# soedinglab/hh-suite

Hardware: NVIDIA H100
Metric: Viterbi GCUPS (query_L x sum target_L / s) (higher is better)
Workload: dtype f32

## Files before the change

### hh-suite_b200/csrc/hhg_api.cu

```cuda
#include "../../include/hhg.h"
#include "hhg_kernels.cuh"
#include "hhg_hhm.cuh"
#include "hhg_msa.cuh"
#include "hhg_crf.cuh"
#include "hhg_mac.cuh"
#include "hhg_topk.cuh"
#include "hhg_hitlist.h"

#include <dlfcn.h>
#if defined(__SSE__)
#include <xmmintrin.h>
#endif

#include <algorithm>
#include <chrono>
#include <atomic>
#include <cstdarg>
#include <cstdio>
#include <cstdlib>
#include <cstring>
#include <memory>
#include <cmath>
#include <cfloat>
#include <mutex>
// ... 82 lines not shown
}

}

struct hhg_ctx {
  int device = 0;
  std::shared_ptr<void> msa_cache;
  std::shared_ptr<void> crf_cache;
  std::shared_ptr<void> msa_rcp;
  cudaStream_t stream = nullptr;
  bool own_stream = false;
  int sm_count = 0;
  long long launches = 0;
  int Lq = 0, R = 0;
  int nq = 0;
  std::vector<int> q_L, q_row0;
  std::vector<float> h_q_pav;
  bool has_q_pav = false;
  DevBuf<float> d_q_pav, d_pb;
  std::vector<int> ex;
  int ex_nq = 0, ex_nt = 0;
  DevBuf<int> d_ex;
  unsigned long long query_serial = 0;
  int group_jobs = 16;
  uint32_t epoch = 0;
  uint32_t epoch_window = 1;
  DevBuf<float4> qrec;
  DevBuf<float> S33;
  DevBuf<float> lg2, diff;
  std::vector<float> h_lg2;
  bool has_ss = false, has_S33 = false;
  hhg_params par{1, 0.f, 0.f, -0.03f, 0.11f, 0, 0.1f, 2};
  DevBuf<uint8_t> pf_prof, sw_prof;
  DevBuf<uint8_t> pf_edge[2];
  DevBuf<int> sw_ids, sw_scores;
  DevBuf<unsigned> pf_counter, pf_hist;
  DevBuf<int> pf_corr, pf_ids_a, pf_score_a, pf_ids_b;
  int mac_Lq = 0;
  DevBuf<float> mac_qp, mac_qtr, mac_ttr, mac_post, mac_out_post;
  DevBuf<uint8_t> mac_off, mac_bt, mac_out_states;
  DevBuf<double> mac_rows, mac_scale;
  DevBuf<long long> mac_i64, mac_dbg;
  DevBuf<int> mac_i32, mac_out_i, mac_out_j, mac_map;
  cudaStream_t aux_stream = nullptr;
  cudaEvent_t aux_ev[2] = {nullptr, nullptr};
  DevBuf<MacHitOut> mac_out;
  std::vector<long long> mac_cell_off;
// ... 113 lines not shown
  c->device = device;
  c->sm_count = prop.multiProcessorCount;
  if (stream) {
    c->stream = (cudaStream_t)stream;
  } else {
    CK(cudaStreamCreateWithFlags(&c->stream, cudaStreamNonBlocking));
    c->own_stream = true;
  }
  c->R = strip_rows();
  {
    std::vector<float> lg2(1025, 0.f), diff(1025, 0.f);
    float prev = 0.0f;
    for (int i = 1; i <= 1024; ++i) {
      lg2[i] = (float)(::log((double)(1024 + i)) * 1.442695041 - 10.0);
      diff[i - 1] = (float)((double)(lg2[i] - prev) * 1.2352E-4);
      prev = lg2[i];
    }
    c->h_lg2 = lg2;
    cudaError_t e1 = c->lg2.alloc(1025), e2 = c->diff.alloc(1025);
    if (e1 != cudaSuccess || e2 != cudaSuccess) return fail(HHG_ENOMEM, "fast_log2 tables");
    CK(cudaMemcpy(c->lg2.p, lg2.data(), 1025 * 4, cudaMemcpyHostToDevice));
    CK(cudaMemcpy(c->diff.p, diff.data(), 1025 * 4, cudaMemcpyHostToDevice));
  }
  { const char* ge = getenv("HHG_GROUP_JOBS"); c->group_jobs = ge ? std::max(1, atoi(ge)) : 16; }
  size_t free_b = 0, total_b = 0;
  CK(cudaMemGetInfo(&free_b, &total_b));
  const char* env = getenv("HHG_MAX_BT_GB");
  double cap = env ? atof(env) * 1e9 : 48e9;
  c->max_bt_bytes = (size_t)std::min(cap, 0.45 * (double)free_b);
  *out = holder.release();
  return HHG_OK;
}

int hhg_ctx_destroy(hhg_ctx* ctx) {
  if (!ctx) return HHG_OK;
  cudaSetDevice(ctx->device);
  if (ctx->scratch_plan) hhg_plan_destroy(ctx->scratch_plan);
  for (auto& e : ctx->ev) if (e) cudaEventDestroy(e);
  for (auto& e : ctx->aux_ev) if (e) cudaEventDestroy(e);
  if (ctx->aux_stream) cudaStreamDestroy(ctx->aux_stream);
  if (ctx->own_stream && ctx->stream) cudaStreamDestroy(ctx->stream);
  delete ctx;
  return HHG_OK;
}

int hhg_ctx_sync(hhg_ctx* ctx) {
  if (!ctx) return fail(HHG_EINVAL, "ctx is NULL");
// ... 1149 lines not shown
      max_wave_words = std::max(max_wave_words, wave_bt);
      w.job_begin = jb;
      wave_bt = 0;
    }
    JobDesc d{};
    d.ss_off = ss; d.bt_off = (long long)wave_bt; d.bnd_off = bnd; d.co_off = co; d.jc_off = jc;
    d.Lmax = Lmax; d.query = q; d.nstrips = ns; d.Lq = ctx->q_L[q]; d.qrow0 = ctx->q_row0[q];
    pl->jobs.push_back(d);
    wave_bt += words;
    bnd += (long long)(Lmax + 1) * 32;
    jc += (long long)Lmax * 224;
    co += (long long)ns * (Lmax + 1) * 32;
    ss += ns;
    pl->padded_cells += (double)ns * R * (double)Lmax * 32.0;
    first += cnt;
  }
  pl->njobs = (int)pl->jobs.size();
  w.job_end = pl->njobs;
  pl->waves.push_back(w);
  max_wave_words = std::max(max_wave_words, wave_bt);
  pl->ss_total = ss;
  pl->co_total = co;
  pl->items.clear();
  for (Wave& wv : pl->waves) {
    wv.item_begin = (long long)pl->items.size();
    for (int g0 = wv.job_begin; g0 < wv.job_end; g0 += ctx->group_jobs) {
      const int g1 = std::min(g0 + ctx->group_jobs, wv.job_end);
      int maxns = 0;
      for (int jb = g0; jb < g1; ++jb) maxns = std::max(maxns, pl->jobs[jb].nstrips);
      for (int sidx = 0; sidx < maxns; ++sidx)
        for (int jb = g0; jb < g1; ++jb)
          if (sidx < pl->jobs[jb].nstrips) pl->items.push_back(make_int2(jb - wv.job_begin, sidx));
    }
    wv.item_end = (long long)pl->items.size();
  }
  long long po = 0;
  double cols_sum = 0;
  for (int k = 0; k < n; ++k) {
    ReqDesc& r = pl->reqs[k];
    r.target = pl->ids[k];
    r.Lt = db->L[r.target];
    r.Lq = ctx->q_L[pl->req_query[k]];
    r.path_off = po;
    po += r.Lq + r.Lt + 2;
    pl->cells += (double)r.Lq * r.Lt;
    cols_sum += r.Lt;
  }
  if (po > 0x7fffffffLL) return fail(HHG_EINVAL, "plan too large: %lld path bytes (> 2^31-1); split the request", po);
  pl->path_total = po;
  pl->jc_total = jc;
  pl->alg_bytes = cols_sum * 112.0 + pl->cells * 1.0 + (double)sizeof(HitRec) * n;

  cudaError_t e = cudaSuccess;
  auto A = [&](cudaError_t r) { if (e == cudaSuccess) e = r; };
  A(pl->d_jobs.ensure(pl->njobs)); A(pl->d_reqs.ensure(n));
  A(pl->d_job_target.ensure(job_target.size())); A(pl->d_items.ensure(pl->items.size()));
  A(pl->d_jcols.ensure((size_t)jc + 224));
// ... 86 lines not shown
    ctx->launches++;
    CK(cudaGetLastError());
    CK(cudaStreamSynchronize(ctx->stream));
  }
  pl->celloff = true;
  pl->n_excl_steps = (int)total;
  return HHG_OK;
}

int hhg_set_excluded_regions(hhg_ctx* ctx, int nq, const int32_t* q_lo, const int32_t* q_hi, int nt, const int32_t* t_lo,
                             const int32_t* t_hi) {
  if (!ctx || nq < 0 || nt < 0 || (nq && (!q_lo || !q_hi)) || (nt && (!t_lo || !t_hi)))
    return fail(HHG_EINVAL, "hhg_set_excluded_regions: bad argument");
  ctx->ex.assign(q_lo, q_lo + nq);
  ctx->ex.insert(ctx->ex.end(), q_hi, q_hi + nq);
  ctx->ex.insert(ctx->ex.end(), t_lo, t_lo + nt);
  ctx->ex.insert(ctx->ex.end(), t_hi, t_hi + nt);
  ctx->ex_nq = nq;
  ctx->ex_nt = nt;
  return HHG_OK;
}

template <int R>
static int launch_viterbi(hhg_ctx* ctx, const VitParams& P, bool local, bool ss, bool co, int items) {
  const size_t smem = (size_t)kWarpsPerCta * (R * 112 + kRingBytes) + 64 + (ss ? 44 * 44 * 4 : 0);
  void (*kern)(const VitParams) = nullptr;
#define PICK(L_, S_, C_) kern = k_viterbi<R, L_, S_, C_>
  if (local) { if (ss) { if (co) PICK(true, true, true); else PICK(true, true, false); }
               else    { if (co) PICK(true, false, true); else PICK(true, false, false); } }
  else       { if (ss) { if (co) PICK(false, true, true); else PICK(false, true, false); }
               else    { if (co) PICK(false, false, true); else PICK(false, false, false); } }
#undef PICK
  CK(cudaFuncSetAttribute(kern, cudaFuncAttributeMaxDynamicSharedMemorySize, (int)smem));
  int per_sm = 0;
  CK(cudaOccupancyMaxActiveBlocksPerMultiprocessor(&per_sm, kern, kWarpsPerCta * 32, smem));
  if (per_sm < 1) return fail(HHG_ECUDA, "viterbi kernel does not fit on an SM");
  int grid = ctx->sm_count * per_sm;
  const int need = (items + kWarpsPerCta - 1) / kWarpsPerCta;
  if (grid > need) grid = need;
  kern<<<grid, kWarpsPerCta * 32, smem, ctx->stream>>>(P);
  ctx->launches++;
  CK(cudaGetLastError());
  return HHG_OK;
}

static int plan_run_impl(hhg_ctx* ctx, hhg_plan* pl, bool timed) {
  if (!ctx || !pl) return fail(HHG_EINVAL, "hhg_plan_run: bad argument");
  if (pl->q_L != ctx->q_L || pl->q_row0 != ctx->q_row0) return fail(HHG_EINVAL, "plan was made for another query (batch) geometry");
  const hhg_db* db = pl->db;
  const bool fused = pl->nm_mode >= 0;
  if (fused && (!db->raw || !ctx->has_q_pav)) return fail(HHG_EINVAL, "fused null model needs a raw shard and query pav");
  if (!fused && !db->prepared) return fail(HHG_EINVAL, "raw db: call hhg_db_apply_null_model for the current query first");
  if (ctx->par.use_ss && (!db->has_ss || !ctx->has_ss || !ctx->has_S33))
    return fail(HHG_EINVAL, "use_ss requested but query/db/S33 carry no ss information");
  CK(cudaSetDevice(ctx->device));
  cudaStream_t st = ctx->stream;
  ctx->epoch = (ctx->epoch + 1) & 0xFFFFFu;
  if (ctx->epoch == 0) { ctx->epoch = 1; ctx->epoch_window++; }
  if (pl->bnd_epoch_window != ctx->epoch_window) {
    if (pl->d_bnd.p) CK(cudaMemsetAsync(pl->d_bnd.p, 0, pl->d_bnd.n * sizeof(BndSlot), st));
    pl->bnd_epoch_window = ctx->epoch_window;
  }
  CK(cudaMemsetAsync(pl->d_counter.p, 0, pl->waves.size() * 4, st));
  if (pl->jc_version != db->cols_version || pl->jc_nm_mode != pl->nm_mode ||
      (fused && pl->jc_query_serial != ctx->query_serial)) {
    int maxL = 0;
    for (const JobDesc& jd : pl->jobs) maxL = std::max(maxL, jd.Lmax);
    dim3 grid((unsigned)pl->njobs, (unsigned)std::min(64, (maxL + 7) / 8), 1);
    k_interleave_cols<<<grid, 256, 0, st>>>(pl->d_jobs.p, pl->d_job_target.p, fused ? db->cols_raw.p : db->cols.p,
                                            db->dcol_off.p, db->dL.p, pl->d_jcols.p, pl->nm_mode, ctx->d_q_pav.p,
                                            db->pav.p, ctx->d_pb.p);
    ctx->launches++;
    CK(cudaGetLastError());
    pl->jc_version = db->cols_version;
    pl->jc_nm_mode = pl->nm_mode;
    pl->jc_query_serial = ctx->query_serial;
  }
  for (size_t wi = 0; wi < pl->waves.size(); ++wi) {
    const Wave& w = pl->waves[wi];
    const int nj = w.job_end - w.job_begin;
    VitParams P{};
    P.qrec = ctx->qrec.p;
    P.jobs = pl->d_jobs.p + w.job_begin;
    P.items = pl->d_items.p + w.item_begin; P.n_items = (int)(w.item_end - w.item_begin);
    P.Lt = db->dL.p;
    P.jcols = pl->d_jcols.p;
    P.njobs = nj;
    P.job_target = pl->d_job_target.p + (size_t)w.job_begin * 32;
    P.bt = pl->d_bt.p; P.bnd = pl->d_bnd.p;
    P.tag_base = ctx->epoch << 12;
    P.counter = pl->d_counter.p + wi;
    P.strip_score = pl->d_strip_score.p;
    P.strip_ij = pl->d_strip_ij.p;
    P.celloff = pl->celloff ? pl->d_co.p : nullptr;
    P.S33 = ctx->has_S33 ? ctx->S33.p : nullptr;
    P.egq = ctx->par.egq; P.egt = ctx->par.egt; P.shift = ctx->par.shift; P.ssw = ctx->par.ssw;
    P.zero = 0u;

    const int items = P.n_items;
    int rc;
    if (timed) CK(cudaEventRecord(ctx->ev[0], st));
    if (pl->R == 8) rc = launch_viterbi<8>(ctx, P, ctx->par.local != 0, ctx->par.use_ss != 0, pl->celloff, items);
    else if (pl->R == 12) rc = launch_viterbi<12>(ctx, P, ctx->par.local != 0, ctx->par.use_ss != 0, pl->celloff, items);
    else rc = launch_viterbi<16>(ctx, P, ctx->par.local != 0, ctx->par.use_ss != 0, pl->celloff, items);
    if (rc != HHG_OK) return rc;
    if (timed) CK(cudaEventRecord(ctx->ev[1], st));
    BtParams B{};
    B.n_req = pl->n;
    B.jobs = pl->d_jobs.p; B.reqs = pl->d_reqs.p;
    B.nm_mode = pl->nm_mode; B.q_pav = ctx->d_q_pav.p; B.t_pav = db->pav.p; B.pb = ctx->d_pb.p;
    B.bt = pl->d_bt.p; B.strip_score = pl->d_strip_score.p; B.strip_ij = pl->d_strip_ij.p;
    B.hits = pl->d_hits.p; B.paths = pl->d_paths.p;
    B.job_begin = w.job_begin; B.job_end = w.job_end;
    B.qrec = ctx->qrec.p; B.cols = fused ? db->cols_raw.p : db->cols.p; B.col_off = db->dcol_off.p;
    B.lg2 = ctx->lg2.p; B.diff = ctx->diff.p; B.S33 = ctx->has_S33 ? ctx->S33.p : nullptr; B.S = pl->d_S.p;
    B.corr = ctx->par.corr; B.ssw = ctx->par.ssw; B.use_ss = ctx->par.use_ss; B.ss_score_mode = (ctx->par.ssm == 2);
    const int threads = 128;
    k_backtrace<<<(pl->n + threads - 1) / threads, threads, 0, st>>>(B);
    ctx->launches++;
    CK(cudaGetLastError());
    if (timed) {
      CK(cudaEventRecord(ctx->ev[2], st));
      CK(cudaEventSynchronize(ctx->ev[2]));
      float a = 0, b = 0;
      CK(cudaEventElapsedTime(&a, ctx->ev[0], ctx->ev[1]));
      CK(cudaEventElapsedTime(&b, ctx->ev[1], ctx->ev[2]));
      pl->ms_viterbi += a;
// ... 851 lines not shown
```

### hh-suite_b200/csrc/hhg_kernels.cuh

```cuda
#pragma once
#include <cuda_runtime.h>
#include <float.h>
#include <stdint.h>

#ifndef HHG_MAX3
#define HHG_MAX3 1
#endif

#include "hhg_math.cuh"

namespace hhg {

constexpr int kWarpsPerCta = 4;

struct __align__(16) ColRec {
  float p[20];
  float m2m, m2d, d2m, d2d, i2m;
  float i2i, m2i;
  uint32_t ss;
};
static_assert(sizeof(ColRec) == 112, "ColRec must be 7 x 16 bytes");

struct __align__(8) BndSlot {
  unsigned long long w[5];
// ... 9 lines not shown
  asm volatile("st.relaxed.gpu.global.v2.b64 [%0], {%1,%2};" ::"l"(p + 2 * lane), "l"(tagged(mm, tag)),
               "l"(tagged(dg, tag)) : "memory");
  asm volatile("st.relaxed.gpu.global.v2.b64 [%0], {%1,%2};" ::"l"(p + 64 + 2 * lane), "l"(tagged(mi, tag)),
               "l"(tagged(gd, tag)) : "memory");
  asm volatile("st.relaxed.gpu.global.b64 [%0], %1;" ::"l"(p + 128 + lane), "l"(tagged(im, tag)) : "memory");
}
__device__ __forceinline__ void ld_slot(const BndSlot* col, int lane, float& mm, float& dg, float& mi, float& gd,
                                        float& im, uint32_t (&tag)[5]) {
  const unsigned long long* p = reinterpret_cast<const unsigned long long*>(col);
  unsigned long long w0, w1, w2, w3, w4;
  asm volatile("ld.relaxed.gpu.global.v2.b64 {%0,%1}, [%2];" : "=l"(w0), "=l"(w1) : "l"(p + 2 * lane) : "memory");
  asm volatile("ld.relaxed.gpu.global.v2.b64 {%0,%1}, [%2];" : "=l"(w2), "=l"(w3) : "l"(p + 64 + 2 * lane) : "memory");
  asm volatile("ld.relaxed.gpu.global.b64 %0, [%1];" : "=l"(w4) : "l"(p + 128 + lane) : "memory");
  mm = __uint_as_float((uint32_t)w0); tag[0] = (uint32_t)(w0 >> 32);
  dg = __uint_as_float((uint32_t)w1); tag[1] = (uint32_t)(w1 >> 32);
  mi = __uint_as_float((uint32_t)w2); tag[2] = (uint32_t)(w2 >> 32);
  gd = __uint_as_float((uint32_t)w3); tag[3] = (uint32_t)(w3 >> 32);
  im = __uint_as_float((uint32_t)w4); tag[4] = (uint32_t)(w4 >> 32);
}
__device__ __forceinline__ bool slot_ok(const uint32_t (&tag)[5], uint32_t want) {
  return ((tag[0] ^ want) | (tag[1] ^ want) | (tag[2] ^ want) | (tag[3] ^ want) | (tag[4] ^ want)) == 0u;
}

struct JobDesc {
  long long ss_off;
  long long bt_off;
  long long bnd_off;
  long long co_off;
  long long jc_off;
  int Lmax;
  int query;
  int nstrips;
  int Lq;
  int qrow0;
};
static_assert(sizeof(JobDesc) == 64, "JobDesc: 5 x int64 + 5 x int32, tail padding only");

struct ReqDesc {
  long long path_off;
  int job;
  int lane;
  int target;
  int Lt;
  int Lq;
};
static_assert(sizeof(ReqDesc) == 32, "ReqDesc: 1 x int64 + 5 x int32, tail padding only");

struct VitParams {
  const float4* qrec;
  const JobDesc* jobs;
  const int2* items;
  int n_items;
  const int* Lt;
  const float4* jcols;
  int njobs;
  const int* job_target;
  uint32_t* bt;
  struct BndSlot* bnd;
  uint32_t tag_base;
  unsigned int* counter;
  float* strip_score;
  int* strip_ij;
  const uint32_t* celloff;
  const float* S33;
  float egq, egt, shift, ssw;
  uint32_t zero;
};

__device__ __forceinline__ uint32_t smem_u32(const void* p) {
// ... 31 lines not shown
  const float e = __fadd_rn(__uint_as_float((u >> 23) | 0x4B000000u), -8388735.0f);
  const float m = __uint_as_float((u & 0x007FFFFFu) | 0x3F800000u);
  float p = -0.107254423828329604454f;
  p = __fadd_rn(__fmul_rn(p, m), 0.688243882994381274313f);
  p = __fadd_rn(__fmul_rn(p, m), -1.75647175389045657003f);
  p = __fadd_rn(__fmul_rn(p, m), 2.61761038894603480148f);
  p = __fmul_rn(p, __fadd_rn(m, -1.0f));
  return __fadd_rn(p, e);
}

__device__ __forceinline__ float dot20_dev(const float4 (&t)[5], const float4 (&q)[5]) {
  float r0 = __fmul_rn(t[0].x, q[0].x), r1 = __fmul_rn(t[0].y, q[0].y);
  float r2 = __fmul_rn(t[0].z, q[0].z), r3 = __fmul_rn(t[0].w, q[0].w);
#pragma unroll
  for (int m = 1; m < 5; ++m) {
    r0 = __fadd_rn(__fmul_rn(t[m].x, q[m].x), r0);
    r1 = __fadd_rn(__fmul_rn(t[m].y, q[m].y), r1);
    r2 = __fadd_rn(__fmul_rn(t[m].z, q[m].z), r2);
    r3 = __fadd_rn(__fmul_rn(t[m].w, q[m].w), r3);
  }
  return __fadd_rn(__fadd_rn(r0, r1), __fadd_rn(r2, r3));
}

__device__ __forceinline__ void cp_async_jc(float4* dst, const float4* src) {
  asm volatile("cp.async.cg.shared.global [%0], [%1], 16;" ::"r"(smem_u32(dst)), "l"(src) : "memory");
}
__device__ __forceinline__ void cp_async_commit() { asm volatile("cp.async.commit_group;" ::: "memory"); }
__device__ __forceinline__ void cp_async_wait_all() { asm volatile("cp.async.wait_all;" ::: "memory"); }

constexpr int kJcSlot = 7 * 32;
constexpr size_t kRingBytes = 2 * kJcSlot * 16;

#define HHG_NEG (-FLT_MAX)

template <int R, bool LOCAL, bool SS, bool CELLOFF>
__global__ void __launch_bounds__(kWarpsPerCta * 32, (R <= 12) ? 3 : 2)
    k_viterbi(const VitParams P) {
  static_assert(R % 4 == 0, "R must be a multiple of 4");
  extern __shared__ __align__(128) unsigned char smem_raw[];
  const int warp = threadIdx.x >> 5;
  const int lane = threadIdx.x & 31;
  float4* qs = reinterpret_cast<float4*>(smem_raw) + (size_t)warp * R * 7;
  constexpr size_t kRingOff = (size_t)kWarpsPerCta * R * 112;
  float4* ring = reinterpret_cast<float4*>(smem_raw + kRingOff + (size_t)warp * kRingBytes) + lane;
  constexpr size_t kBarOff = kRingOff + kWarpsPerCta * kRingBytes;
  uint64_t* bars = reinterpret_cast<uint64_t*>(smem_raw + kBarOff);
  float* s33 = reinterpret_cast<float*>(smem_raw + kBarOff + 64);
  uint64_t* bar = bars + warp;

  if (lane == 0) mbar_init(bar, 1);
  if (SS) {
    for (int k = threadIdx.x; k < 44 * 44; k += blockDim.x) s33[k] = P.S33[k];
  }
  asm volatile("fence.mbarrier_init.release.cluster;" ::: "memory");
  __syncthreads();

  const float smin = LOCAL ? 0.0f : HHG_NEG;
  const int total_items = P.n_items;
  uint32_t parity = 0;

  for (;;) {
    int item = 0;
    if (lane == 0) item = (int)atomicAdd(P.counter, 1u);
    item = __shfl_sync(0xffffffffu, item, 0);
    if (item >= total_items) break;
    const int2 it = __ldg(P.items + item);
    const int job = it.x, s = it.y;
    const JobDesc* jd = P.jobs + job;
    const int Lq = jd->Lq;
    const int nstrips = jd->nstrips;
    const int i0 = s * R;

    if (lane == 0) {
      mbar_expect_tx(bar, R * 112);
      tma_bulk_g2s(qs, P.qrec + (size_t)(jd->qrow0 + i0) * 7, R * 112, bar);
    }

    const int t = P.job_target[job * 32 + lane];
    const int Lt = P.Lt[t];
    const int Lmax = jd->Lmax;
    const float4* jc = P.jcols + jd->jc_off + lane;
    const size_t bt_row_stride = (size_t)(Lmax + 1) * 32;
    uint32_t* btc = P.bt + jd->bt_off + lane + (size_t)(i0 >> 2) * bt_row_stride + 32;
    BndSlot* bndc = P.bnd + jd->bnd_off + 32;
    const uint32_t tag_in = P.tag_base + (uint32_t)s;
    const uint32_t tag_out = P.tag_base + (uint32_t)s + 1u;
    const bool last_strip = (s == nstrips - 1);
    const uint32_t* co = nullptr;
    if (CELLOFF) co = P.celloff + jd->co_off + (size_t)s * (Lmax + 1) * 32 + lane + 32;

    float MM[R], GD[R], IM[R], DG[R], Y[R];
#pragma unroll
    for (int r = 0; r < R; ++r) {
      MM[r] = __fmul_rn((float)(-(i0 + 1 + r)), P.egq);
      GD[r] = IM[r] = DG[r] = HHG_NEG;
    }
    float dtMM = __fmul_rn((float)(-i0), P.egq), dtDG = HHG_NEG, dtGD = HHG_NEG, dtIM = HHG_NEG;

    float best = HHG_NEG;
    int bi = 0, bj = 0;

#pragma unroll
    for (int k = 0; k < 7; ++k) cp_async_jc(ring + k * 32, jc + k * 32);
    cp_async_commit();
    int rd = 0;

    float nMM = 0.f, nDG = 0.f, nMI = 0.f, nGD = 0.f, nIM = 0.f;
    uint32_t ntag[5] = {0u, 0u, 0u, 0u, 0u};
    if (s > 0) ld_slot(bndc, lane, nMM, nDG, nMI, nGD, nIM, ntag);

    mbar_wait(bar, parity);
    parity ^= 1u;
#pragma unroll
    for (int r = 0; r < R; ++r) Y[r] = __fadd_rn(HHG_NEG, qs[r * 7 + 5].x);

    for (int j = 1; j <= Lmax; ++j) {
      cp_async_wait_all();
      const float4* cur = ring + rd;
      const float4 tp[5] = {cur[0], cur[32], cur[64], cur[96], cur[128]};
      const float4 tt0 = cur[160], tt1 = cur[192];
      const float t_m2m = tt0.x, t_m2d = tt0.y, t_d2m = tt0.z, t_d2d = tt0.w;
      const float t_i2m = tt1.x, t_i2i = tt1.y, t_m2i = tt1.z;
      const uint32_t t_ss = __float_as_uint(tt1.w);
      rd ^= kJcSlot;
      jc += 224;
#pragma unroll
      for (int k = 0; k < 7; ++k) cp_async_jc(ring + rd + k * 32, jc + k * 32);
      cp_async_commit();

      float tMM, tDG, tMI, tGD, tIM;
      if (s == 0) {
        tMM = __fmul_rn((float)(-j), P.egt);
        tDG = tMI = tGD = tIM = HHG_NEG;
      } else {
        if (!__all_sync(0xffffffffu, slot_ok(ntag, tag_in))) {
          while (!slot_ok(ntag, tag_in)) {
            __nanosleep(20);
            ld_slot(bndc, lane, nMM, nDG, nMI, nGD, nIM, ntag);
          }
        }
        tMM = nMM; tDG = nDG; tMI = nMI; tGD = nGD; tIM = nIM;
        ld_slot(bndc + 32, lane, nMM, nDG, nMI, nGD, nIM, ntag);
      }
      uint32_t cow = 0;
      if (CELLOFF) cow = __ldg(co);

      float4 qa = qs[5], qb = qs[6];
      float pMM = __fadd_rn(dtMM, qa.x), pGD = __fadd_rn(dtGD, qa.x), pIM = __fadd_rn(dtIM, qb.x),
            pDG = __fadd_rn(dtDG, qa.z);
      float uMM = tMM, uDG = tDG, uMI = tMI;
      const float bcmp = (j <= Lt) ? best : INFINITY;
      float bc = bcmp;

      uint32_t word = SS ? 0u : (t_ss & P.zero);
#pragma unroll
      for (int r = 0; r < R; ++r) {
        float4 q[5];
#pragma unroll
        for (int k = 0; k < 5; ++k) q[k] = qs[r * 7 + k];
        const float q_m2m = qa.x, q_m2d = qa.y, q_d2m = qa.z, q_d2d = qa.w;
        const float q_i2m = qb.x, q_i2i = qb.y, q_m2i = qb.z;

        uint32_t b;
        float mm;
        const float c1 = __fadd_rn(pMM, t_m2m);
        const float c2 = __fadd_rn(pGD, t_d2m);
        const float c3 = __fadd_rn(pIM, t_m2m);
        const float c4 = __fadd_rn(pDG, t_m2m);
        const float c5 = __fadd_rn(Y[r], t_i2m);
#if HHG_MAX3
        mm = fmaxf(fmaxf(smin, c1), c2);
        mm = fmaxf(fmaxf(mm, c3), c4);
        mm = fmaxf(mm, c5);
        b = 6u;
        b = (c4 == mm) ? 5u : b;
        b = (c3 == mm) ? 4u : b;
        b = (c2 == mm) ? 3u : b;
        b = (c1 == mm) ? 2u : b;
        b = (smin == mm) ? 0u : b;
#else
        b = (c1 > smin) ? 2u : 0u; mm = fmaxf(smin, c1);
        b = (c2 > mm) ? 3u : b;    mm = fmaxf(mm, c2);
        b = (c3 > mm) ? 4u : b;    mm = fmaxf(mm, c3);
        b = (c4 > mm) ? 5u : b;    mm = fmaxf(mm, c4);
        b = (c5 > mm) ? 6u : b;    mm = fmaxf(mm, c5);
#endif

        float Si = log2f4_dev(dot20_dev(tp, q));
        if (SS) {
          const uint32_t q_ss = __float_as_uint(qb.w);
          Si = __fadd_rn(__fmul_rn(P.ssw, s33[q_ss * 44 + t_ss]), Si);
        }
        Si = __fadd_rn(Si, P.shift);
        mm = __fadd_rn(mm, Si);

        const float oMM = MM[r], oGD = GD[r], oIM = IM[r], oDG = DG[r];
        float a1, a2, gd, im, dg, mi;
        a1 = __fadd_rn(oMM, t_m2d); a2 = __fadd_rn(oGD, t_d2d);
        b |= (a1 > a2) ? 8u : 0u;  gd = fmaxf(a1, a2);
        a1 = __fadd_rn(__fadd_rn(oMM, q_m2i), t_m2m); a2 = __fadd_rn(__fadd_rn(oIM, q_i2i), t_m2m);
        b |= (a1 > a2) ? 16u : 0u; im = fmaxf(a1, a2);
        a1 = __fadd_rn(uMM, q_m2d); a2 = __fadd_rn(uDG, q_d2d);
        b |= (a1 > a2) ? 32u : 0u; dg = fmaxf(a1, a2);
        Y[r] = __fadd_rn(uMI, q_m2m);
        a1 = __fadd_rn(__fadd_rn(uMM, q_m2m), t_m2i); a2 = __fadd_rn(Y[r], t_i2i);
        b |= (a1 > a2) ? 64u : 0u; mi = fmaxf(a1, a2);

        if (CELLOFF) {
          const float off = ((cow >> r) & 1u) ? HHG_NEG : 0.0f;
          mm = __fadd_rn(mm, off); gd = __fadd_rn(gd, off); im = __fadd_rn(im, off);
          dg = __fadd_rn(dg, off); mi = __fadd_rn(mi, off);
        }

        word |= b << (8 * (r & 3));
        if ((r & 3) == 3) {
          __stcs(btc + (size_t)(r >> 2) * bt_row_stride, word);
          word = 0;
        }
        if (r + 1 < R) {
          qa = qs[(r + 1) * 7 + 5]; qb = qs[(r + 1) * 7 + 6];
          pMM = __fadd_rn(oMM, qa.x); pGD = __fadd_rn(oGD, qa.x); pIM = __fadd_rn(oIM, qb.x);
          pDG = __fadd_rn(oDG, qa.z);
        }
        uMM = mm; uDG = dg; uMI = mi;
        MM[r] = mm; GD[r] = gd; IM[r] = im; DG[r] = dg;
      }
      dtMM = tMM; dtDG = tDG; dtGD = tGD; dtIM = tIM;

      {
        float c0 = MM[0], c1 = MM[1], c2 = MM[2], c3 = MM[3];
#pragma unroll
        for (int r = 4; r < R; r += 4) {
          c0 = fmaxf(c0, MM[r]); c1 = fmaxf(c1, MM[r + 1]); c2 = fmaxf(c2, MM[r + 2]); c3 = fmaxf(c3, MM[r + 3]);
        }
        if (fmaxf(fmaxf(c0, c1), fmaxf(c2, c3)) >= bc) {
#pragma unroll
          for (int r = 0; r < R; ++r) {
            const float mm = MM[r];
            if (mm >= bc) {
              const int i = i0 + 1 + r;
              const bool cand = (i <= Lq) && (LOCAL || i == Lq || j == Lt);
              if (cand && (mm > best || i < bi)) { best = mm; bi = i; bj = j; bc = mm; }
            }
          }
        }
      }

      if (!last_strip) st_slot(bndc, lane, uMM, uDG, uMI, GD[R - 1], IM[R - 1], tag_out);
      bndc += 32;
      btc += 32;
      if (CELLOFF) co += 32;
    }
    int jb = job;
    asm("" : "+r"(jb));
    const size_t o = ((size_t)P.jobs[jb].ss_off + s) * 32 + lane;
    P.strip_score[o] = best;
    P.strip_ij[o] = (bi << 16) | bj;
    cp_async_wait_all();
    __syncwarp();
  }
}

__device__ __forceinline__ void null_model_vec(int columnscore, const float* __restrict__ q_pav,
                                               const float* __restrict__ t_pav, const float* __restrict__ pb,
                                               float (&pn)[20]) {
#pragma unroll
  for (int a = 0; a < 20; ++a) {
    switch (columnscore) {
      case 0: pn[a] = pb[a]; break;
      case 2: pn[a] = t_pav[a]; break;
      case 3: pn[a] = q_pav[a]; break;
      default: pn[a] = __fmul_rn(0.5f, __fadd_rn(q_pav[a], t_pav[a])); break;
    }
  }
}
__device__ __forceinline__ float4 div4(float4 v, const float* pn) {
  v.x = __fdiv_rn(v.x, pn[0]); v.y = __fdiv_rn(v.y, pn[1]); v.z = __fdiv_rn(v.z, pn[2]); v.w = __fdiv_rn(v.w, pn[3]);
  return v;
}

struct HitRec {
  float score;
// ... 462 lines not shown
```

Measured before the change: 191.6.

## Hand off strip boundaries between warps via shared-memory mbarrier rings

Work is now scheduled per CTA in quads of consecutive strips of the same job. Adjacent warps pass boundary column values through a shared-memory ring guarded by mbarriers, replacing the global-memory tagged boundary slots and polling. The plan builder groups strips into CTA-sized runs with padding, the default group size rises from 16 to 256, and cp.async switches from .cg to .ca. The cost is extra shared memory per CTA, possible idle warps from padding, and a __syncthreads per quad that ties warps together.

```diff
diff --git a/hh-suite_b200/csrc/hhg_api.cu b/hh-suite_b200/csrc/hhg_api.cu
--- a/hh-suite_b200/csrc/hhg_api.cu
+++ b/hh-suite_b200/csrc/hhg_api.cu
@@ -128,7 +128,7 @@
   int ex_nq = 0, ex_nt = 0;
   DevBuf<int> d_ex;
   unsigned long long query_serial = 0;
-  int group_jobs = 16;
+  int group_jobs = 256;
   uint32_t epoch = 0;
   uint32_t epoch_window = 1;
   DevBuf<float4> qrec;
@@ -288,7 +288,7 @@
     CK(cudaMemcpy(c->lg2.p, lg2.data(), 1025 * 4, cudaMemcpyHostToDevice));
     CK(cudaMemcpy(c->diff.p, diff.data(), 1025 * 4, cudaMemcpyHostToDevice));
   }
-  { const char* ge = getenv("HHG_GROUP_JOBS"); c->group_jobs = ge ? std::max(1, atoi(ge)) : 16; }
+  { const char* ge = getenv("HHG_GROUP_JOBS"); c->group_jobs = ge ? std::max(1, atoi(ge)) : 256; }
   size_t free_b = 0, total_b = 0;
   CK(cudaMemGetInfo(&free_b, &total_b));
   const char* env = getenv("HHG_MAX_BT_GB");
@@ -1484,17 +1484,31 @@
   pl->ss_total = ss;
   pl->co_total = co;
   pl->items.clear();
+  auto push_run = [&](int jb, int s0, int cnt) {
+    for (int k = 0; k < cnt; ++k)
+      pl->items.push_back(make_int2(jb, (s0 + k) | (k > 0 ? kFromWarp : 0) | (k + 1 < cnt ? kToWarp : 0)));
+  };
+  auto pad_quad = [&] {
+    while (pl->items.size() % kWarpsPerCta) pl->items.push_back(make_int2(-1, 0));
+  };
   for (Wave& wv : pl->waves) {
-    wv.item_begin = (long long)pl->items.size();
+    wv.item_begin = (long long)pl->items.size() / kWarpsPerCta;
     for (int g0 = wv.job_begin; g0 < wv.job_end; g0 += ctx->group_jobs) {
       const int g1 = std::min(g0 + ctx->group_jobs, wv.job_end);
-      int maxns = 0;
-      for (int jb = g0; jb < g1; ++jb) maxns = std::max(maxns, pl->jobs[jb].nstrips);
-      for (int sidx = 0; sidx < maxns; ++sidx)
+      int maxq = 0;
+      for (int jb = g0; jb < g1; ++jb) maxq = std::max(maxq, pl->jobs[jb].nstrips / kWarpsPerCta);
+      for (int q = 0; q < maxq; ++q)
         for (int jb = g0; jb < g1; ++jb)
-          if (sidx < pl->jobs[jb].nstrips) pl->items.push_back(make_int2(jb - wv.job_begin, sidx));
+          if (q < pl->jobs[jb].nstrips / kWarpsPerCta) push_run(jb - wv.job_begin, q * kWarpsPerCta, kWarpsPerCta);
+      for (int jb = g0; jb < g1; ++jb) {
+        const int ns = pl->jobs[jb].nstrips, rem = ns % kWarpsPerCta;
+        if (rem == 0) continue;
+        if ((int)(pl->items.size() % kWarpsPerCta) + rem > kWarpsPerCta) pad_quad();
+        push_run(jb - wv.job_begin, ns - rem, rem);
+      }
+      pad_quad();
     }
-    wv.item_end = (long long)pl->items.size();
+    wv.item_end = (long long)pl->items.size() / kWarpsPerCta;
   }
   long long po = 0;
   double cols_sum = 0;
@@ -1627,8 +1641,8 @@
 }
 
 template <int R>
-static int launch_viterbi(hhg_ctx* ctx, const VitParams& P, bool local, bool ss, bool co, int items) {
-  const size_t smem = (size_t)kWarpsPerCta * (R * 112 + kRingBytes) + 64 + (ss ? 44 * 44 * 4 : 0);
+static int launch_viterbi(hhg_ctx* ctx, const VitParams& P, bool local, bool ss, bool co, int quads) {
+  const size_t smem = vit_smem_bytes(R, ss);
   void (*kern)(const VitParams) = nullptr;
 #define PICK(L_, S_, C_) kern = k_viterbi<R, L_, S_, C_>
   if (local) { if (ss) { if (co) PICK(true, true, true); else PICK(true, true, false); }
@@ -1641,8 +1655,7 @@
   CK(cudaOccupancyMaxActiveBlocksPerMultiprocessor(&per_sm, kern, kWarpsPerCta * 32, smem));
   if (per_sm < 1) return fail(HHG_ECUDA, "viterbi kernel does not fit on an SM");
   int grid = ctx->sm_count * per_sm;
-  const int need = (items + kWarpsPerCta - 1) / kWarpsPerCta;
-  if (grid > need) grid = need;
+  if (grid > quads) grid = quads;
   kern<<<grid, kWarpsPerCta * 32, smem, ctx->stream>>>(P);
   ctx->launches++;
   CK(cudaGetLastError());
@@ -1687,7 +1700,7 @@
     VitParams P{};
     P.qrec = ctx->qrec.p;
     P.jobs = pl->d_jobs.p + w.job_begin;
-    P.items = pl->d_items.p + w.item_begin; P.n_items = (int)(w.item_end - w.item_begin);
+    P.items = pl->d_items.p + w.item_begin * kWarpsPerCta; P.n_items = (int)(w.item_end - w.item_begin);
     P.Lt = db->dL.p;
     P.jcols = pl->d_jcols.p;
     P.njobs = nj;
@@ -1702,12 +1715,12 @@
     P.egq = ctx->par.egq; P.egt = ctx->par.egt; P.shift = ctx->par.shift; P.ssw = ctx->par.ssw;
     P.zero = 0u;
 
-    const int items = P.n_items;
+    const int quads = P.n_items;
     int rc;
     if (timed) CK(cudaEventRecord(ctx->ev[0], st));
-    if (pl->R == 8) rc = launch_viterbi<8>(ctx, P, ctx->par.local != 0, ctx->par.use_ss != 0, pl->celloff, items);
-    else if (pl->R == 12) rc = launch_viterbi<12>(ctx, P, ctx->par.local != 0, ctx->par.use_ss != 0, pl->celloff, items);
-    else rc = launch_viterbi<16>(ctx, P, ctx->par.local != 0, ctx->par.use_ss != 0, pl->celloff, items);
+    if (pl->R == 8) rc = launch_viterbi<8>(ctx, P, ctx->par.local != 0, ctx->par.use_ss != 0, pl->celloff, quads);
+    else if (pl->R == 12) rc = launch_viterbi<12>(ctx, P, ctx->par.local != 0, ctx->par.use_ss != 0, pl->celloff, quads);
+    else rc = launch_viterbi<16>(ctx, P, ctx->par.local != 0, ctx->par.use_ss != 0, pl->celloff, quads);
     if (rc != HHG_OK) return rc;
     if (timed) CK(cudaEventRecord(ctx->ev[1], st));
     BtParams B{};
diff --git a/hh-suite_b200/csrc/hhg_kernels.cuh b/hh-suite_b200/csrc/hhg_kernels.cuh
--- a/hh-suite_b200/csrc/hhg_kernels.cuh
+++ b/hh-suite_b200/csrc/hhg_kernels.cuh
@@ -55,6 +55,19 @@
   return ((tag[0] ^ want) | (tag[1] ^ want) | (tag[2] ^ want) | (tag[3] ^ want) | (tag[4] ^ want)) == 0u;
 }
 
+constexpr int kHandCols = 8;
+struct HandCol {
+  float4 a[32];
+  float b[32];
+};
+struct HandRing {
+  HandCol col[kHandCols];
+  uint64_t full[kHandCols], empty[kHandCols];
+};
+static_assert(sizeof(HandRing) == 5248, "HandRing: 8 x 640 B columns + 16 mbarriers");
+__host__ __device__ constexpr uint32_t hand_full(uint32_t c) { return kHandCols * sizeof(HandCol) + 8 * c; }
+__host__ __device__ constexpr uint32_t hand_empty(uint32_t c) { return (kHandCols * sizeof(HandCol)) + 8 * (kHandCols + c); }
+
 struct JobDesc {
   long long ss_off;
   long long bt_off;
@@ -78,6 +91,10 @@
   int Lq;
 };
 static_assert(sizeof(ReqDesc) == 32, "ReqDesc: 1 x int64 + 5 x int32, tail padding only");
+
+constexpr int kFromWarp = 1 << 30;
+constexpr int kToWarp = 1 << 29;
+constexpr int kStripMask = kToWarp - 1;
 
 struct VitParams {
   const float4* qrec;
@@ -155,14 +172,42 @@
   return __fadd_rn(__fadd_rn(r0, r1), __fadd_rn(r2, r3));
 }
 
+__device__ __forceinline__ bool mbar_test_a(uint32_t bar, uint32_t parity) {
+  uint32_t ok;
+  asm volatile("{ .reg .pred p; mbarrier.test_wait.parity.shared::cta.b64 p, [%1], %2; selp.u32 %0, 1, 0, p; }"
+               : "=r"(ok) : "r"(bar), "r"(parity) : "memory");
+  return ok != 0;
+}
+__device__ __forceinline__ void mbar_wait_a(uint32_t bar, uint32_t parity) {
+  while (!mbar_test_a(bar, parity)) __nanosleep(20);
+}
+__device__ __forceinline__ void mbar_arrive_a(uint32_t bar) {
+  asm volatile("mbarrier.arrive.shared::cta.b64 _, [%0];" ::"r"(bar) : "memory");
+}
+__device__ __forceinline__ void hand_put(uint32_t col, int lane, float mm, float dg, float mi, float gd, float im) {
+  asm volatile("st.shared.v4.f32 [%0], {%1,%2,%3,%4};" ::"r"(col + 16 * lane), "f"(mm), "f"(dg), "f"(mi), "f"(gd)
+               : "memory");
+  asm volatile("st.shared.f32 [%0], %1;" ::"r"(col + 512 + 4 * lane), "f"(im) : "memory");
+}
+__device__ __forceinline__ void hand_get(uint32_t col, int lane, float& mm, float& dg, float& mi, float& gd, float& im) {
+  asm volatile("ld.shared.v4.f32 {%0,%1,%2,%3}, [%4];" : "=f"(mm), "=f"(dg), "=f"(mi), "=f"(gd) : "r"(col + 16 * lane)
+               : "memory");
+  asm volatile("ld.shared.f32 %0, [%1];" : "=f"(im) : "r"(col + 512 + 4 * lane) : "memory");
+}
+
 __device__ __forceinline__ void cp_async_jc(float4* dst, const float4* src) {
-  asm volatile("cp.async.cg.shared.global [%0], [%1], 16;" ::"r"(smem_u32(dst)), "l"(src) : "memory");
+  asm volatile("cp.async.ca.shared.global [%0], [%1], 16;" ::"r"(smem_u32(dst)), "l"(src) : "memory");
 }
 __device__ __forceinline__ void cp_async_commit() { asm volatile("cp.async.commit_group;" ::: "memory"); }
 __device__ __forceinline__ void cp_async_wait_all() { asm volatile("cp.async.wait_all;" ::: "memory"); }
 
 constexpr int kJcSlot = 7 * 32;
 constexpr size_t kRingBytes = 2 * kJcSlot * 16;
+
+__host__ __device__ constexpr size_t vit_smem_bytes(int R, bool ss) {
+  return (size_t)kWarpsPerCta * (R * 112 + kRingBytes) + 64 + (kWarpsPerCta - 1) * sizeof(HandRing) +
+         (ss ? 44 * 44 * 4 : 0);
+}
 
 #define HHG_NEG (-FLT_MAX)
 
@@ -178,10 +223,21 @@
   float4* ring = reinterpret_cast<float4*>(smem_raw + kRingOff + (size_t)warp * kRingBytes) + lane;
   constexpr size_t kBarOff = kRingOff + kWarpsPerCta * kRingBytes;
   uint64_t* bars = reinterpret_cast<uint64_t*>(smem_raw + kBarOff);
-  float* s33 = reinterpret_cast<float*>(smem_raw + kBarOff + 64);
+  volatile int* quad_idx = reinterpret_cast<volatile int*>(smem_raw + kBarOff + 32);
+  HandRing* hands = reinterpret_cast<HandRing*>(smem_raw + kBarOff + 64);
+  float* s33 = reinterpret_cast<float*>(hands + (kWarpsPerCta - 1));
   uint64_t* bar = bars + warp;
+  HandRing* hin = reinterpret_cast<HandRing*>(smem_raw + kBarOff + 64 - sizeof(HandRing)) + warp;
+  const uint32_t hin_a = smem_u32(hin);
+  uint32_t hin_n = 0, hout_n = 0;
 
   if (lane == 0) mbar_init(bar, 1);
+  if (threadIdx.x < (kWarpsPerCta - 1) * kHandCols) {
+    HandRing& h = hands[threadIdx.x / kHandCols];
+    mbar_init(&h.full[threadIdx.x % kHandCols], 32);
+    mbar_init(&h.empty[threadIdx.x % kHandCols], 32);
+  }
+  if (threadIdx.x == 0) quad_idx[0] = (int)atomicAdd(P.counter, 1u);
   if (SS) {
     for (int k = threadIdx.x; k < 44 * 44; k += blockDim.x) s33[k] = P.S33[k];
   }
@@ -192,205 +248,221 @@
   const int total_items = P.n_items;
   uint32_t parity = 0;
 
-  for (;;) {
-    int item = 0;
-    if (lane == 0) item = (int)atomicAdd(P.counter, 1u);
-    item = __shfl_sync(0xffffffffu, item, 0);
-    if (item >= total_items) break;
-    const int2 it = __ldg(P.items + item);
-    const int job = it.x, s = it.y;
-    const JobDesc* jd = P.jobs + job;
-    const int Lq = jd->Lq;
-    const int nstrips = jd->nstrips;
-    const int i0 = s * R;
-
-    if (lane == 0) {
-      mbar_expect_tx(bar, R * 112);
-      tma_bulk_g2s(qs, P.qrec + (size_t)(jd->qrow0 + i0) * 7, R * 112, bar);
-    }
-
-    const int t = P.job_target[job * 32 + lane];
-    const int Lt = P.Lt[t];
-    const int Lmax = jd->Lmax;
-    const float4* jc = P.jcols + jd->jc_off + lane;
-    const size_t bt_row_stride = (size_t)(Lmax + 1) * 32;
-    uint32_t* btc = P.bt + jd->bt_off + lane + (size_t)(i0 >> 2) * bt_row_stride + 32;
-    BndSlot* bndc = P.bnd + jd->bnd_off + 32;
-    const uint32_t tag_in = P.tag_base + (uint32_t)s;
-    const uint32_t tag_out = P.tag_base + (uint32_t)s + 1u;
-    const bool last_strip = (s == nstrips - 1);
-    const uint32_t* co = nullptr;
-    if (CELLOFF) co = P.celloff + jd->co_off + (size_t)s * (Lmax + 1) * 32 + lane + 32;
-
-    float MM[R], GD[R], IM[R], DG[R], Y[R];
-#pragma unroll
-    for (int r = 0; r < R; ++r) {
-      MM[r] = __fmul_rn((float)(-(i0 + 1 + r)), P.egq);
-      GD[r] = IM[r] = DG[r] = HHG_NEG;
-    }
-    float dtMM = __fmul_rn((float)(-i0), P.egq), dtDG = HHG_NEG, dtGD = HHG_NEG, dtIM = HHG_NEG;
-
-    float best = HHG_NEG;
-    int bi = 0, bj = 0;
-
-#pragma unroll
-    for (int k = 0; k < 7; ++k) cp_async_jc(ring + k * 32, jc + k * 32);
-    cp_async_commit();
-    int rd = 0;
-
-    float nMM = 0.f, nDG = 0.f, nMI = 0.f, nGD = 0.f, nIM = 0.f;
-    uint32_t ntag[5] = {0u, 0u, 0u, 0u, 0u};
-    if (s > 0) ld_slot(bndc, lane, nMM, nDG, nMI, nGD, nIM, ntag);
-
-    mbar_wait(bar, parity);
-    parity ^= 1u;
-#pragma unroll
-    for (int r = 0; r < R; ++r) Y[r] = __fadd_rn(HHG_NEG, qs[r * 7 + 5].x);
-
-    for (int j = 1; j <= Lmax; ++j) {
-      cp_async_wait_all();
-      const float4* cur = ring + rd;
-      const float4 tp[5] = {cur[0], cur[32], cur[64], cur[96], cur[128]};
-      const float4 tt0 = cur[160], tt1 = cur[192];
-      const float t_m2m = tt0.x, t_m2d = tt0.y, t_d2m = tt0.z, t_d2d = tt0.w;
-      const float t_i2m = tt1.x, t_i2i = tt1.y, t_m2i = tt1.z;
-      const uint32_t t_ss = __float_as_uint(tt1.w);
-      rd ^= kJcSlot;
-      jc += 224;
-#pragma unroll
-      for (int k = 0; k < 7; ++k) cp_async_jc(ring + rd + k * 32, jc + k * 32);
+  for (int qb = 0;; qb ^= 1) {
+    const int quad = quad_idx[qb];
+    if (quad >= total_items) break;
+    if (threadIdx.x == 0) quad_idx[qb ^ 1] = (int)atomicAdd(P.counter, 1u);
+    const int2 it = __ldg(P.items + (size_t)quad * kWarpsPerCta + warp);
+    if (it.x >= 0) {
+      const int job = it.x, s = it.y & kStripMask;
+      const bool from_warp = (it.y & kFromWarp) != 0, to_warp = (it.y & kToWarp) != 0;
+      const JobDesc* jd = P.jobs + job;
+      const int Lq = jd->Lq;
+      const int nstrips = jd->nstrips;
+      const int i0 = s * R;
+
+      if (lane == 0) {
+        mbar_expect_tx(bar, R * 112);
+        tma_bulk_g2s(qs, P.qrec + (size_t)(jd->qrow0 + i0) * 7, R * 112, bar);
+      }
+
+      const int t = P.job_target[job * 32 + lane];
+      const int Lt = P.Lt[t];
+      const int Lmax = jd->Lmax;
+      const float4* jc = P.jcols + jd->jc_off + lane;
+      const size_t bt_row_stride = (size_t)(Lmax + 1) * 32;
+      uint32_t* btc = P.bt + jd->bt_off + lane + (size_t)(i0 >> 2) * bt_row_stride + 32;
+      BndSlot* bndc = P.bnd + jd->bnd_off + 32;
+      const uint32_t tag_in = P.tag_base + (uint32_t)s;
+      const uint32_t tag_out = P.tag_base + (uint32_t)s + 1u;
+      const bool last_strip = (s == nstrips - 1);
+      const uint32_t* co = nullptr;
+      if (CELLOFF) co = P.celloff + jd->co_off + (size_t)s * (Lmax + 1) * 32 + lane + 32;
+
+      float MM[R], GD[R], IM[R], DG[R], Y[R];
+#pragma unroll
+      for (int r = 0; r < R; ++r) {
+        MM[r] = __fmul_rn((float)(-(i0 + 1 + r)), P.egq);
+        GD[r] = IM[r] = DG[r] = HHG_NEG;
+      }
+      float dtMM = __fmul_rn((float)(-i0), P.egq), dtDG = HHG_NEG, dtGD = HHG_NEG, dtIM = HHG_NEG;
+
+      float best = HHG_NEG;
+      int bi = 0, bj = 0;
+
+#pragma unroll
+      for (int k = 0; k < 7; ++k) cp_async_jc(ring + k * 32, jc + k * 32);
       cp_async_commit();
-
-      float tMM, tDG, tMI, tGD, tIM;
-      if (s == 0) {
-        tMM = __fmul_rn((float)(-j), P.egt);
-        tDG = tMI = tGD = tIM = HHG_NEG;
-      } else {
-        if (!__all_sync(0xffffffffu, slot_ok(ntag, tag_in))) {
-          while (!slot_ok(ntag, tag_in)) {
-            __nanosleep(20);
-            ld_slot(bndc, lane, nMM, nDG, nMI, nGD, nIM, ntag);
+      int rd = 0;
+
+      float nMM = 0.f, nDG = 0.f, nMI = 0.f, nGD = 0.f, nIM = 0.f;
+      uint32_t ntag[5] = {0u, 0u, 0u, 0u, 0u};
+      if (s > 0 && !from_warp) ld_slot(bndc, lane, nMM, nDG, nMI, nGD, nIM, ntag);
+
+      mbar_wait(bar, parity);
+      parity ^= 1u;
+#pragma unroll
+      for (int r = 0; r < R; ++r) Y[r] = __fadd_rn(HHG_NEG, qs[r * 7 + 5].x);
+
+      for (int j = 1; j <= Lmax; ++j) {
+        cp_async_wait_all();
+        const float4* cur = ring + rd;
+        const float4 tp[5] = {cur[0], cur[32], cur[64], cur[96], cur[128]};
+        const float4 tt0 = cur[160], tt1 = cur[192];
+        const float t_m2m = tt0.x, t_m2d = tt0.y, t_d2m = tt0.z, t_d2d = tt0.w;
+        const float t_i2m = tt1.x, t_i2i = tt1.y, t_m2i = tt1.z;
+        const uint32_t t_ss = __float_as_uint(tt1.w);
+        rd ^= kJcSlot;
+        jc += 224;
+#pragma unroll
+        for (int k = 0; k < 7; ++k) cp_async_jc(ring + rd + k * 32, jc + k * 32);
+        cp_async_commit();
+
+        float tMM, tDG, tMI, tGD, tIM;
+        if (s == 0) {
+          tMM = __fmul_rn((float)(-j), P.egt);
+          tDG = tMI = tGD = tIM = HHG_NEG;
+        } else if (from_warp) {
+          const uint32_t slot = hin_n % kHandCols;
+          mbar_wait_a(hin_a + hand_full(slot), (hin_n / kHandCols) & 1u);
+          hand_get(hin_a + slot * sizeof(HandCol), lane, tMM, tDG, tMI, tGD, tIM);
+          mbar_arrive_a(hin_a + hand_empty(slot));
+          ++hin_n;
+        } else {
+          if (!__all_sync(0xffffffffu, slot_ok(ntag, tag_in))) {
+            while (!slot_ok(ntag, tag_in)) {
+              __nanosleep(20);
+              ld_slot(bndc, lane, nMM, nDG, nMI, nGD, nIM, ntag);
+            }
           }
+          tMM = nMM; tDG = nDG; tMI = nMI; tGD = nGD; tIM = nIM;
+          ld_slot(bndc + 32, lane, nMM, nDG, nMI, nGD, nIM, ntag);
         }
-        tMM = nMM; tDG = nDG; tMI = nMI; tGD = nGD; tIM = nIM;
-        ld_slot(bndc + 32, lane, nMM, nDG, nMI, nGD, nIM, ntag);
-      }
-      uint32_t cow = 0;
-      if (CELLOFF) cow = __ldg(co);
-
-      float4 qa = qs[5], qb = qs[6];
-      float pMM = __fadd_rn(dtMM, qa.x), pGD = __fadd_rn(dtGD, qa.x), pIM = __fadd_rn(dtIM, qb.x),
-            pDG = __fadd_rn(dtDG, qa.z);
-      float uMM = tMM, uDG = tDG, uMI = tMI;
-      const float bcmp = (j <= Lt) ? best : INFINITY;
-      float bc = bcmp;
-
-      uint32_t word = SS ? 0u : (t_ss & P.zero);
-#pragma unroll
-      for (int r = 0; r < R; ++r) {
-        float4 q[5];
-#pragma unroll
-        for (int k = 0; k < 5; ++k) q[k] = qs[r * 7 + k];
-        const float q_m2m = qa.x, q_m2d = qa.y, q_d2m = qa.z, q_d2d = qa.w;
-        const float q_i2m = qb.x, q_i2i = qb.y, q_m2i = qb.z;
-
-        uint32_t b;
-        float mm;
-        const float c1 = __fadd_rn(pMM, t_m2m);
-        const float c2 = __fadd_rn(pGD, t_d2m);
-        const float c3 = __fadd_rn(pIM, t_m2m);
-        const float c4 = __fadd_rn(pDG, t_m2m);
-        const float c5 = __fadd_rn(Y[r], t_i2m);
+        uint32_t cow = 0;
+        if (CELLOFF) cow = __ldg(co);
+
+        float4 qa = qs[5], qb = qs[6];
+        float pMM = __fadd_rn(dtMM, qa.x), pGD = __fadd_rn(dtGD, qa.x), pIM = __fadd_rn(dtIM, qb.x),
+              pDG = __fadd_rn(dtDG, qa.z);
+        float uMM = tMM, uDG = tDG, uMI = tMI;
+        const float bcmp = (j <= Lt) ? best : INFINITY;
+        float bc = bcmp;
+
+        uint32_t word = SS ? 0u : (t_ss & P.zero);
+#pragma unroll
+        for (int r = 0; r < R; ++r) {
+          float4 q[5];
+#pragma unroll
+          for (int k = 0; k < 5; ++k) q[k] = qs[r * 7 + k];
+          const float q_m2m = qa.x, q_m2d = qa.y, q_d2m = qa.z, q_d2d = qa.w;
+          const float q_i2m = qb.x, q_i2i = qb.y, q_m2i = qb.z;
+
+          uint32_t b;
+          float mm;
+          const float c1 = __fadd_rn(pMM, t_m2m);
+          const float c2 = __fadd_rn(pGD, t_d2m);
+          const float c3 = __fadd_rn(pIM, t_m2m);
+          const float c4 = __fadd_rn(pDG, t_m2m);
+          const float c5 = __fadd_rn(Y[r], t_i2m);
 #if HHG_MAX3
-        mm = fmaxf(fmaxf(smin, c1), c2);
-        mm = fmaxf(fmaxf(mm, c3), c4);
-        mm = fmaxf(mm, c5);
-        b = 6u;
-        b = (c4 == mm) ? 5u : b;
-        b = (c3 == mm) ? 4u : b;
-        b = (c2 == mm) ? 3u : b;
-        b = (c1 == mm) ? 2u : b;
-        b = (smin == mm) ? 0u : b;
+          mm = fmaxf(fmaxf(smin, c1), c2);
+          mm = fmaxf(fmaxf(mm, c3), c4);
+          mm = fmaxf(mm, c5);
+          b = 6u;
+          b = (c4 == mm) ? 5u : b;
+          b = (c3 == mm) ? 4u : b;
+          b = (c2 == mm) ? 3u : b;
+          b = (c1 == mm) ? 2u : b;
+          b = (smin == mm) ? 0u : b;
 #else
-        b = (c1 > smin) ? 2u : 0u; mm = fmaxf(smin, c1);
-        b = (c2 > mm) ? 3u : b;    mm = fmaxf(mm, c2);
-        b = (c3 > mm) ? 4u : b;    mm = fmaxf(mm, c3);
-        b = (c4 > mm) ? 5u : b;    mm = fmaxf(mm, c4);
-        b = (c5 > mm) ? 6u : b;    mm = fmaxf(mm, c5);
+          b = (c1 > smin) ? 2u : 0u; mm = fmaxf(smin, c1);
+          b = (c2 > mm) ? 3u : b;    mm = fmaxf(mm, c2);
+          b = (c3 > mm) ? 4u : b;    mm = fmaxf(mm, c3);
+          b = (c4 > mm) ? 5u : b;    mm = fmaxf(mm, c4);
+          b = (c5 > mm) ? 6u : b;    mm = fmaxf(mm, c5);
 #endif
 
-        float Si = log2f4_dev(dot20_dev(tp, q));
-        if (SS) {
-          const uint32_t q_ss = __float_as_uint(qb.w);
-          Si = __fadd_rn(__fmul_rn(P.ssw, s33[q_ss * 44 + t_ss]), Si);
+          float Si = log2f4_dev(dot20_dev(tp, q));
+          if (SS) {
+            const uint32_t q_ss = __float_as_uint(qb.w);
+            Si = __fadd_rn(__fmul_rn(P.ssw, s33[q_ss * 44 + t_ss]), Si);
+          }
+          Si = __fadd_rn(Si, P.shift);
+          mm = __fadd_rn(mm, Si);
+
+          const float oMM = MM[r], oGD = GD[r], oIM = IM[r], oDG = DG[r];
+          float a1, a2, gd, im, dg, mi;
+          a1 = __fadd_rn(oMM, t_m2d); a2 = __fadd_rn(oGD, t_d2d);
+          b |= (a1 > a2) ? 8u : 0u;  gd = fmaxf(a1, a2);
+          a1 = __fadd_rn(__fadd_rn(oMM, q_m2i), t_m2m); a2 = __fadd_rn(__fadd_rn(oIM, q_i2i), t_m2m);
+          b |= (a1 > a2) ? 16u : 0u; im = fmaxf(a1, a2);
+          a1 = __fadd_rn(uMM, q_m2d); a2 = __fadd_rn(uDG, q_d2d);
+          b |= (a1 > a2) ? 32u : 0u; dg = fmaxf(a1, a2);
+          Y[r] = __fadd_rn(uMI, q_m2m);
+          a1 = __fadd_rn(__fadd_rn(uMM, q_m2m), t_m2i); a2 = __fadd_rn(Y[r], t_i2i);
+          b |= (a1 > a2) ? 64u : 0u; mi = fmaxf(a1, a2);
+
+          if (CELLOFF) {
+            const float off = ((cow >> r) & 1u) ? HHG_NEG : 0.0f;
+            mm = __fadd_rn(mm, off); gd = __fadd_rn(gd, off); im = __fadd_rn(im, off);
+            dg = __fadd_rn(dg, off); mi = __fadd_rn(mi, off);
+          }
+
+          word |= b << (8 * (r & 3));
+          if ((r & 3) == 3) {
+            __stcs(btc + (size_t)(r >> 2) * bt_row_stride, word);
+            word = 0;
+          }
+          if (r + 1 < R) {
+            qa = qs[(r + 1) * 7 + 5]; qb = qs[(r + 1) * 7 + 6];
+            pMM = __fadd_rn(oMM, qa.x); pGD = __fadd_rn(oGD, qa.x); pIM = __fadd_rn(oIM, qb.x);
+            pDG = __fadd_rn(oDG, qa.z);
+          }
+          uMM = mm; uDG = dg; uMI = mi;
+          MM[r] = mm; GD[r] = gd; IM[r] = im; DG[r] = dg;
         }
-        Si = __fadd_rn(Si, P.shift);
-        mm = __fadd_rn(mm, Si);
-
-        const float oMM = MM[r], oGD = GD[r], oIM = IM[r], oDG = DG[r];
-        float a1, a2, gd, im, dg, mi;
-        a1 = __fadd_rn(oMM, t_m2d); a2 = __fadd_rn(oGD, t_d2d);
-        b |= (a1 > a2) ? 8u : 0u;  gd = fmaxf(a1, a2);
-        a1 = __fadd_rn(__fadd_rn(oMM, q_m2i), t_m2m); a2 = __fadd_rn(__fadd_rn(oIM, q_i2i), t_m2m);
-        b |= (a1 > a2) ? 16u : 0u; im = fmaxf(a1, a2);
-        a1 = __fadd_rn(uMM, q_m2d); a2 = __fadd_rn(uDG, q_d2d);
-        b |= (a1 > a2) ? 32u : 0u; dg = fmaxf(a1, a2);
-        Y[r] = __fadd_rn(uMI, q_m2m);
-        a1 = __fadd_rn(__fadd_rn(uMM, q_m2m), t_m2i); a2 = __fadd_rn(Y[r], t_i2i);
-        b |= (a1 > a2) ? 64u : 0u; mi = fmaxf(a1, a2);
-
-        if (CELLOFF) {
-          const float off = ((cow >> r) & 1u) ? HHG_NEG : 0.0f;
-          mm = __fadd_rn(mm, off); gd = __fadd_rn(gd, off); im = __fadd_rn(im, off);
-          dg = __fadd_rn(dg, off); mi = __fadd_rn(mi, off);
-        }
-
-        word |= b << (8 * (r & 3));
-        if ((r & 3) == 3) {
-          __stcs(btc + (size_t)(r >> 2) * bt_row_stride, word);
-          word = 0;
-        }
-        if (r + 1 < R) {
-          qa = qs[(r + 1) * 7 + 5]; qb = qs[(r + 1) * 7 + 6];
-          pMM = __fadd_rn(oMM, qa.x); pGD = __fadd_rn(oGD, qa.x); pIM = __fadd_rn(oIM, qb.x);
-          pDG = __fadd_rn(oDG, qa.z);
-        }
-        uMM = mm; uDG = dg; uMI = mi;
-        MM[r] = mm; GD[r] = gd; IM[r] = im; DG[r] = dg;
-      }
-      dtMM = tMM; dtDG = tDG; dtGD = tGD; dtIM = tIM;
-
-      {
-        float c0 = MM[0], c1 = MM[1], c2 = MM[2], c3 = MM[3];
-#pragma unroll
-        for (int r = 4; r < R; r += 4) {
-          c0 = fmaxf(c0, MM[r]); c1 = fmaxf(c1, MM[r + 1]); c2 = fmaxf(c2, MM[r + 2]); c3 = fmaxf(c3, MM[r + 3]);
-        }
-        if (fmaxf(fmaxf(c0, c1), fmaxf(c2, c3)) >= bc) {
-#pragma unroll
-          for (int r = 0; r < R; ++r) {
-            const float mm = MM[r];
-            if (mm >= bc) {
-              const int i = i0 + 1 + r;
-              const bool cand = (i <= Lq) && (LOCAL || i == Lq || j == Lt);
-              if (cand && (mm > best || i < bi)) { best = mm; bi = i; bj = j; bc = mm; }
+        dtMM = tMM; dtDG = tDG; dtGD = tGD; dtIM = tIM;
+
+        {
+          float c0 = MM[0], c1 = MM[1], c2 = MM[2], c3 = MM[3];
+#pragma unroll
+          for (int r = 4; r < R; r += 4) {
+            c0 = fmaxf(c0, MM[r]); c1 = fmaxf(c1, MM[r + 1]); c2 = fmaxf(c2, MM[r + 2]); c3 = fmaxf(c3, MM[r + 3]);
+          }
+          if (fmaxf(fmaxf(c0, c1), fmaxf(c2, c3)) >= bc) {
+#pragma unroll
+            for (int r = 0; r < R; ++r) {
+              const float mm = MM[r];
+              if (mm >= bc) {
+                const int i = i0 + 1 + r;
+                const bool cand = (i <= Lq) && (LOCAL || i == Lq || j == Lt);
+                if (cand && (mm > best || i < bi)) { best = mm; bi = i; bj = j; bc = mm; }
+              }
             }
           }
         }
+
+        if (to_warp) {
+          const uint32_t slot = hout_n % kHandCols, hout_a = hin_a + sizeof(HandRing);
+          mbar_wait_a(hout_a + hand_empty(slot), ((hout_n / kHandCols) & 1u) ^ 1u);
+          hand_put(hout_a + slot * sizeof(HandCol), lane, uMM, uDG, uMI, GD[R - 1], IM[R - 1]);
+          mbar_arrive_a(hout_a + hand_full(slot));
+          ++hout_n;
+        } else if (!last_strip) {
+          st_slot(bndc, lane, uMM, uDG, uMI, GD[R - 1], IM[R - 1], tag_out);
+        }
+        bndc += 32;
+        btc += 32;
+        if (CELLOFF) co += 32;
       }
-
-      if (!last_strip) st_slot(bndc, lane, uMM, uDG, uMI, GD[R - 1], IM[R - 1], tag_out);
-      bndc += 32;
-      btc += 32;
-      if (CELLOFF) co += 32;
+      int jb = job;
+      asm("" : "+r"(jb));
+      const size_t o = ((size_t)P.jobs[jb].ss_off + s) * 32 + lane;
+      P.strip_score[o] = best;
+      P.strip_ij[o] = (bi << 16) | bj;
+      cp_async_wait_all();
     }
-    int jb = job;
-    asm("" : "+r"(jb));
-    const size_t o = ((size_t)P.jobs[jb].ss_off + s) * 32 + lane;
-    P.strip_score[o] = best;
-    P.strip_ij[o] = (bi << 16) | bj;
-    cp_async_wait_all();
-    __syncwarp();
+    __syncthreads();
   }
 }
 
```

Result: faster. 194.1 (median of 6 runs) (+1.3%).
